# prestodb/presto

Measured on AMD Instinct MI355X. Metric: tpch_lineitem_rows_per_sec, higher is better.
Workload: dtype f64; 1 GPU; TPC-H SF100 Q1 & Q3 on 1xMI355X - one step = one Q1 pass + one Q3 pass, columns resident in HBM; query=q1+q3, rows_per_gpu=1200075804, mode=f64

## Files before the change

### include/presto_gpu.h

```cpp
#ifndef PRESTO_GPU_H
#define PRESTO_GPU_H
#include <stdint.h>

#ifdef __cplusplus
extern "C" {
#endif

#define PG_ABI_VERSION 1

typedef int32_t pg_status;
#define PG_OK 0
#define PG_ERR (-1)
const char* pg_last_error(void);

pg_status pg_device_count(int32_t* out);
pg_status pg_device_sync(void);
pg_status pg_device_malloc(int64_t bytes, void** out);
pg_status pg_device_free(void* p);
pg_status pg_memcpy_h2d(void* dst, const void* src, int64_t bytes);
pg_status pg_memcpy_d2h(void* dst, const void* src, int64_t bytes);
pg_status pg_memcpy_d2d(void* dst, const void* src, int64_t bytes);
double pg_last_hot_kernel_ms(void);
double pg_hot_max_ms(void);
void pg_hot_reset(void);
int64_t pg_q1_fast_launches(void);

typedef enum {
    PG_T_U8 = 0,
    PG_T_I32 = 1,
    PG_T_I64 = 2,
    PG_T_F64 = 3,
    PG_T_I128 = 5,
    PG_T_VARBIN = 4,
} pg_type;

typedef struct {
    int32_t tag;
    int32_t on_device;
    void* data;
    const uint8_t* null_mask;
    const int32_t* offsets;
    const int32_t* dict_ids;
    int32_t dict_n;
} pg_col;

typedef struct {
    int64_t n_rows;
    int32_t n_cols;
    pg_col cols[32];
} pg_page;


typedef enum { PG_CMP_LT = 0, PG_CMP_LE, PG_CMP_GT, PG_CMP_GE, PG_CMP_EQ,
               PG_CMP_NE,
               PG_CMP_CONTAINS, PG_CMP_PREFIX,
               PG_CMP_CONTAINS2, PG_CMP_NOT_CONTAINS2,
               PG_CMP_IS_NULL, PG_CMP_IS_NOT_NULL } pg_cmp;

typedef struct {
    int32_t col;
    int32_t op;
    int64_t ival;
    double dval;
    char sval[40];
    int32_t slen;
    int32_t rhs_col;
} pg_pred;

typedef enum {
    PG_PROJ_IDENT = 0,
    PG_PROJ_DISC_PRICE = 1,
    PG_PROJ_CHARGE = 2,
    PG_PROJ_MUL = 3,
    PG_PROJ_DIV = 4,
    PG_PROJ_KEYSHL = 5,
    PG_PROJ_SHR = 6,
    PG_PROJ_SUBDIV = 7,
    PG_PROJ_KEYSHL_DIV = 8,
} pg_proj_kind;

typedef struct {
    int32_t kind;
    int32_t a, b, c;
} pg_proj;

typedef enum {
    PG_AGG_COUNT = 0,
    PG_AGG_SUM_F64 = 1,
    PG_AGG_SUM_DEC = 2,
    PG_AGG_SUM_I64 = 3,
    PG_AGG_MIN = 4,
    PG_AGG_MAX = 5,
} pg_agg_func;

typedef struct {
    int32_t func;
    pg_proj proj;
    int32_t dec_scale;
} pg_agg;

typedef enum {
    PG_OP_FILTER_PROJECT = 1,
    PG_OP_HASH_AGG_SMALL = 2,
    PG_OP_HASH_BUILD = 3,
    PG_OP_LOOKUP_JOIN = 4,
    PG_OP_TOPN = 5,
    PG_OP_PARTITION = 6,
    PG_OP_GROUPBY_MULTI = 7,
    PG_OP_ORDER_BY = 8,
    PG_OP_WINDOW = 10,
} pg_op_kind;

#define PG_MAX_PRED 8
#define PG_MAX_AGG 8
#define PG_MAX_KEYVALS 8

typedef struct {
    int32_t n_preds;
    pg_pred preds[PG_MAX_PRED];
    int32_t n_proj;
    pg_proj proj[16];
    int64_t semijoin_table;
    int32_t semijoin_col;
    int32_t semijoin_anti;
} pg_plan_filter_project;

typedef struct {
    int32_t n_preds;
    pg_pred preds[PG_MAX_PRED];
    int32_t n_keys;
    int32_t key_col[2];
    int32_t n_vals[2];
    uint8_t key_vals[2][PG_MAX_KEYVALS];
    int32_t n_aggs;
    pg_agg aggs[PG_MAX_AGG];
    int32_t drop_unlisted_keys;
} pg_plan_hash_agg_small;

typedef struct {
    int32_t n_preds;
    pg_pred preds[PG_MAX_PRED];
    int32_t key_col;
    int64_t semijoin_table;
    int32_t semijoin_col;
    int32_t n_payload;
    int32_t payload_col[4];
    int64_t capacity_hint;
    int32_t key_set_only;
    int32_t dense_array;
    int64_t payload_lookup_table;
    int32_t payload_lookup_key_col;
    int32_t agg_table;
    int32_t pack_bits;
    int32_t fill_x10;
    int64_t bitmap_max_key;
    int32_t range_group;
    int32_t dense_payload_bias;
} pg_plan_hash_build;

#define PG_JOIN_INNER 0
#define PG_JOIN_PROBE_OUTER 4
#define PG_JOIN_LOOKUP_OUTER 5
#define PG_JOIN_FULL_OUTER 6

typedef struct {
    int64_t table;
    int32_t n_preds;
    pg_pred preds[PG_MAX_PRED];
    int32_t key_col;
    int32_t mode;
    int32_t n_emit;
    int32_t emit_probe_cols[8];
    pg_proj proj;
    int32_t dec_scale;
    int64_t table2;
    int32_t table2_key_col;
    int32_t n_group_vals;
    uint8_t group_vals[8];
// ... 110 lines not shown
```

### presto_amd/csrc/kernels.hip

```cpp
#include <hip/hip_runtime.h>
#include <stdio.h>
#include <stdlib.h>
#include <string.h>
#include <map>
#include <vector>
#include <algorithm>
#include <type_traits>
#include <stdexcept>
#include <string>

#include "../../include/presto_gpu.h"
#include "fixed128.h"
#include "sortkey.h"

static __thread char g_err[512];
extern "C" const char* pg_last_error(void) { return g_err; }
static pg_status seterr(const char* msg)
{
    snprintf(g_err, sizeof(g_err), "%s", msg);
    return PG_ERR;
}
#define CHK(x)                                                          \
    do {                                                                \
        hipError_t e_ = (x);                                            \
        if (e_ != hipSuccess) {                                         \
            snprintf(g_err, sizeof(g_err), "%s:%d %s", __FILE__,        \
                     __LINE__, hipGetErrorString(e_));                  \
            return PG_ERR;                                              \
        }                                                               \
    } while (0)
#define CHKV(x)                                                         \
    do {                                                                \
        hipError_t e_ = (x);                                            \
        if (e_ != hipSuccess) {                                         \
            snprintf(g_err, sizeof(g_err), "%s:%d %s", __FILE__,        \
                     __LINE__, hipGetErrorString(e_));                  \
            throw std::runtime_error(g_err);                            \
        }                                                               \
    } while (0)

static hipStream_t g_stream = nullptr;
static bool g_have_gpu = false;
static pg_status ensure_gpu()
{
    static int state = 0;
    if (state == 0) {
        int n = 0;
        hipError_t e = hipGetDeviceCount(&n);
        if (e != hipSuccess || n == 0) {
            state = -1;
        } else {
            if (hipStreamCreateWithFlags(&g_stream, hipStreamNonBlocking) !=
                hipSuccess)
                state = -1;
            else
                state = 1;
        }
    }
    g_have_gpu = state == 1;
    if (state != 1)
        return seterr("presto_gpu: no AMD GPU available — this library has "
                      "no CPU fallback");
    return PG_OK;
}

extern "C" pg_status pg_device_count(int32_t* out)
{
    int n = 0;
    if (hipGetDeviceCount(&n) != hipSuccess) n = 0;
    *out = n;
    return PG_OK;
}
extern "C" pg_status pg_device_sync(void)
{
    if (ensure_gpu()) return PG_ERR;
    CHK(hipDeviceSynchronize());
    return PG_OK;
}
extern "C" pg_status pg_device_malloc(int64_t bytes, void** out)
{
    if (ensure_gpu()) return PG_ERR;
    CHK(hipMalloc(out, (size_t)bytes));
    return PG_OK;
}
extern "C" pg_status pg_device_free(void* p)
{
    if (ensure_gpu()) return PG_ERR;
    CHK(hipFree(p));
    return PG_OK;
}
extern "C" pg_status pg_memcpy_h2d(void* d, const void* s, int64_t n)
{
    if (ensure_gpu()) return PG_ERR;
    CHK(hipMemcpy(d, s, (size_t)n, hipMemcpyHostToDevice));
    return PG_OK;
}
extern "C" pg_status pg_memcpy_d2h(void* d, const void* s, int64_t n)
{
    if (ensure_gpu()) return PG_ERR;
    CHK(hipMemcpy(d, s, (size_t)n, hipMemcpyDeviceToHost));
    return PG_OK;
}
extern "C" pg_status pg_memcpy_d2d(void* d, const void* s, int64_t n)
{
    if (ensure_gpu()) return PG_ERR;
    CHK(hipMemcpy(d, s, (size_t)n, hipMemcpyDeviceToDevice));
    return PG_OK;
}

static double g_last_hot_ms = 0.0;
static double g_hot_max_ms = 0.0;
static hipEvent_t g_ev0, g_ev1;
static bool g_ev_init = false;
static void hot_begin()
{
    hipError_t e;
    if (!g_ev_init) {
        e = hipEventCreate(&g_ev0);
        e = hipEventCreate(&g_ev1);
        g_ev_init = true;
    }
    e = hipEventRecord(g_ev0, g_stream);
    (void)e;
}
static void hot_end()
{
    hipError_t e;
    e = hipEventRecord(g_ev1, g_stream);
    e = hipEventSynchronize(g_ev1);
    float ms = 0;
    e = hipEventElapsedTime(&ms, g_ev0, g_ev1);
    (void)e;
    g_last_hot_ms = ms;
    if (ms > g_hot_max_ms) g_hot_max_ms = ms;
}
extern "C" double pg_last_hot_kernel_ms(void) { return g_last_hot_ms; }
extern "C" double pg_hot_max_ms(void) { return g_hot_max_ms; }
extern "C" void pg_hot_reset(void) { g_hot_max_ms = 0.0; }
static int64_t g_q1_fast_launches = 0;
extern "C" int64_t pg_q1_fast_launches(void) { return g_q1_fast_launches; }

#define WAVE 64
#define FT_NBLOCKS 4096
#define FT_NTHREADS 256
#define FT_VL ((int64_t)FT_NBLOCKS * FT_NTHREADS)
static const int64_t TBL_EMPTY = INT64_MIN;

__device__ __host__ inline uint8_t d_tbl_tag(uint64_t h)
{
    return (uint8_t)((h >> 56) | 1);
}

__device__ inline double d_load_f64(const pg_col& c, int64_t i)
{
    switch (c.tag) {
        case PG_T_F64: return ((const double*)c.data)[i];
        case PG_T_I64: return (double)((const int64_t*)c.data)[i];
        case PG_T_I32: return (double)((const int32_t*)c.data)[i];
        default: return (double)((const uint8_t*)c.data)[i];
    }
}
__device__ inline int64_t d_load_i64(const pg_col& c, int64_t i)
{
    switch (c.tag) {
        case PG_T_I64: return ((const int64_t*)c.data)[i];
        case PG_T_I32: return (int64_t)((const int32_t*)c.data)[i];
        case PG_T_U8: return (int64_t)((const uint8_t*)c.data)[i];
        default: return (int64_t)((const double*)c.data)[i];
    }
}

__device__ inline int32_t d_find(const uint8_t* d, int32_t n,
                                 const char* pat, int32_t len,
                                 int32_t from)
{
    if (len <= 0) return from <= n ? from : -1;
    const uint8_t c0 = (uint8_t)pat[0];
    const uint32_t c4 = 0x01010101u * c0;
    int32_t last = n - len;
    int32_t s = from;
    for (; s + 3 <= last; ) {
        uint32_t w;
        memcpy(&w, d + s, 4);
        uint32_t x = w ^ c4;
        uint32_t t = (x - 0x01010101u) & ~x & 0x80808080u;
        if (!t) {
            s += 4;
            continue;
        }
        for (int k = 0; k < 4; k++, s++) {
            if (((w >> (8 * k)) & 0xff) != c0) continue;
            bool e = true;
            for (int j = 1; j < len; j++)
                e = e && d[s + j] == (uint8_t)pat[j];
            if (e) return s;
        }
    }
    for (; s <= last; s++) {
        if (d[s] != c0) continue;
        bool e = true;
        for (int j = 1; j < len; j++)
            e = e && d[s + j] == (uint8_t)pat[j];
        if (e) return s;
    }
    return -1;
}

template <bool NULL_TESTS = true>
__device__ inline bool d_eval_preds(const pg_page& pg, const pg_pred* preds,
                                    int n_preds, int64_t i)
{
    for (int p = 0; p < n_preds; p++) {
        const pg_pred& pr = preds[p];
        const pg_col& c = pg.cols[pr.col];
        if constexpr (NULL_TESTS) {
            if (pr.op >= PG_CMP_IS_NULL) {
                const bool is_null = c.null_mask && c.null_mask[i];
                if (is_null != (pr.op == PG_CMP_IS_NULL)) return false;
                continue;
            }
        }
        if (c.null_mask && c.null_mask[i]) return false;
        bool ok;
        if (c.tag == PG_T_VARBIN) {
            int64_t e = c.dict_ids ? (int64_t)c.dict_ids[i] : i;
            int32_t b0 = c.offsets[e], b1 = c.offsets[e + 1];
            const uint8_t* d = (const uint8_t*)c.data + b0;
            int32_t n = b1 - b0;
            if (pr.op == PG_CMP_CONTAINS) {
                ok = d_find(d, n, pr.sval, pr.slen, 0) >= 0;
            } else if (pr.op == PG_CMP_PREFIX) {
                bool e = pr.slen <= n;
                for (int j = 0; e && j < pr.slen; j++)
                    e = d[j] == (uint8_t)pr.sval[j];
                ok = e;
            } else if (pr.op == PG_CMP_CONTAINS2 ||
                       pr.op == PG_CMP_NOT_CONTAINS2) {
                int32_t la = pr.slen, lb = (int32_t)pr.ival;
                int32_t a = d_find(d, n, pr.sval, la, 0);
                bool m = a >= 0 &&
                         d_find(d, n, pr.sval + la, lb, a + la) >= 0;
                ok = (pr.op == PG_CMP_CONTAINS2) ? m : !m;
            } else {
                bool eq = n == pr.slen;
                for (int j = 0; eq && j < pr.slen; j++)
                    eq = d[j] == (uint8_t)pr.sval[j];
                ok = pr.op == PG_CMP_EQ ? eq : !eq;
            }
        } else if (c.tag == PG_T_F64) {
            double v = ((const double*)c.data)[i];
            double x;
            if (pr.rhs_col > 0) {
                const pg_col& rc = pg.cols[pr.rhs_col - 1];
                if (rc.null_mask && rc.null_mask[i]) return false;
                x = d_load_f64(rc, i) + pr.dval;
            } else {
                x = pr.dval;
            }
            switch (pr.op) {
                case PG_CMP_LT: ok = v < x; break;
                case PG_CMP_LE: ok = v <= x; break;
                case PG_CMP_GT: ok = v > x; break;
                case PG_CMP_GE: ok = v >= x; break;
                case PG_CMP_EQ: ok = v == x; break;
                default: ok = v != x; break;
            }
        } else {
            int64_t v = d_load_i64(c, i);
            int64_t x;
            if (pr.rhs_col > 0) {
                const pg_col& rc = pg.cols[pr.rhs_col - 1];
                if (rc.null_mask && rc.null_mask[i]) return false;
                x = d_load_i64(rc, i) + pr.ival;
            } else {
                x = pr.ival;
            }
            switch (pr.op) {
                case PG_CMP_LT: ok = v < x; break;
                case PG_CMP_LE: ok = v <= x; break;
                case PG_CMP_GT: ok = v > x; break;
                case PG_CMP_GE: ok = v >= x; break;
                case PG_CMP_EQ: ok = v == x; break;
                default: ok = v != x; break;
            }
        }
        if (!ok) return false;
    }
    return true;
}

__device__ inline double d_eval_proj_f64(const pg_page& pg, const pg_proj& p,
                                         int64_t i)
{
// ... 835 lines not shown
    int64_t i = (int64_t)blockIdx.x * blockDim.x + threadIdx.x;
    int64_t stride = (int64_t)gridDim.x * blockDim.x;
    for (; i < n; i += stride) {
        int64_t key = in_keys[i];
        if (kbits) {
            if ((uint64_t)(key - 1) >= (uint64_t)bmax) {
                atomicAdd(bm_err, 1ull);
                continue;
            }
            d_kbit_set(kbits, key);
        }
        uint64_t h = pg_murmur3_finalize(pg_bigint_hash(key));
        int64_t s = (int64_t)(h & (uint64_t)mask);
        for (;;) {
            int64_t old = atomicCAS((unsigned long long*)&keys[s],
                                    (unsigned long long)TBL_EMPTY,
                                    (unsigned long long)key);
            if (old == TBL_EMPTY || old == key) {
                if (tags) tags[s] = d_tbl_tag(h);
                int32_t prev = atomicExch(&head[s], (int32_t)i);
                next[i] = prev;
                break;
            }
            s = (s + 1) & mask;
        }
    }
}

__device__ inline int64_t d_probe_next(int64_t s, int64_t lmask)
{
    return (s & ~lmask) | ((s + 1) & lmask);
}

__device__ inline int64_t d_tbl_find_tagged(const int64_t* keys,
                                            const uint8_t* tags,
                                            int64_t mask, int64_t lmask,
                                            int32_t pbits, int64_t key);

struct direct_payloads {
    void* ptr[4];
    int32_t tag[4];
    int32_t src[4];
    int32_t n;
};
__global__ __launch_bounds__(256) void k_tbl_insert_direct(
    pg_page pg, pg_plan_hash_build plan, const int64_t* set_keys,
    int64_t set_mask, const int64_t* lu_keys, const uint8_t* lu_tags,
    int64_t lu_mask, int64_t lu_lmask, const uint8_t* lu_payload,
    int64_t* keys, uint8_t* tags, direct_payloads dp, int64_t mask,
    unsigned long long* inserted, unsigned long long* overflow,
    unsigned long long* pack_err, unsigned long long* kbits, int64_t bmax,
    unsigned long long* bm_err)
{
    const int32_t pbits = plan.pack_bits;
    int64_t i = (int64_t)blockIdx.x * blockDim.x + threadIdx.x;
    int64_t stride = (int64_t)gridDim.x * blockDim.x;
    int64_t my_inserted = 0, my_overflow = 0, my_packerr = 0;
    for (; i < pg.n_rows; i += stride) {
        if (!d_eval_preds<false>(pg, plan.preds, plan.n_preds, i)) continue;
        uint8_t plv = 0;
        if (lu_payload) {
            int64_t k2 =
                d_load_i64(pg.cols[plan.payload_lookup_key_col], i);
            int64_t sl2;
            if (lu_keys) {
                sl2 = d_tbl_find_tagged(lu_keys, lu_tags, lu_mask,
                                        lu_lmask, 0, k2);
            } else {
                sl2 = (k2 >= 1 && k2 <= lu_mask) ? k2 - 1 : -1;
            }
            if (sl2 < 0) continue;
            plv = lu_payload[sl2];
        }
        if (set_keys) {
            int64_t sk = d_load_i64(pg.cols[plan.semijoin_col], i);
            bool found;
            if (set_mask < 0) {
                found = sk >= 1 && sk <= -set_mask &&
                        ((const uint8_t*)set_keys)[sk - 1];
            } else {
                found = false;
                uint64_t h = pg_murmur3_finalize(pg_bigint_hash(sk));
                int64_t s = (int64_t)(h & (uint64_t)set_mask);
                for (;;) {
                    int64_t k = set_keys[s];
                    if (k == sk) { found = true; break; }
                    if (k == TBL_EMPTY) break;
                    s = (s + 1) & set_mask;
                }
            }
            if (!found) continue;
        }
        int64_t key = d_load_i64(pg.cols[plan.key_col], i);
        int64_t word = key;
        if (pbits) {
            int64_t pay0 = lu_payload
                               ? (int64_t)plv
                               : d_load_i64(pg.cols[dp.src[0]], i);
            if (key < 0 || key >= (1ll << (63 - pbits)) || pay0 < 0 ||
                pay0 >= (1ll << pbits)) {
                my_packerr++;
                continue;
            }
            word = (key << pbits) | pay0;
        }
        if (kbits) {
            if ((uint64_t)(key - 1) >= (uint64_t)bmax) {
                atomicAdd(bm_err, 1ull);
                continue;
            }
            d_kbit_set(kbits, key);
        }
        uint64_t h = pg_murmur3_finalize(pg_bigint_hash(key));
        int64_t s = (int64_t)(h & (uint64_t)mask);
        int64_t tries = 0;
        for (;;) {
            int64_t old = atomicCAS((unsigned long long*)&keys[s],
                                    (unsigned long long)TBL_EMPTY,
                                    (unsigned long long)word);
            if (old == TBL_EMPTY || old == word) {
                if (old == TBL_EMPTY) {
                    my_inserted++;
                    if (tags) tags[s] = d_tbl_tag(h);
                }
                if (pbits) break;
                if (lu_payload && dp.n >= 1)
                    ((uint8_t*)dp.ptr[0])[s] = plv;
                for (int o = lu_payload ? 1 : 0; o < dp.n; o++) {
                    const pg_col& c = pg.cols[dp.src[o]];
                    switch (dp.tag[o]) {
                        case PG_T_U8:
                            ((uint8_t*)dp.ptr[o])[s] =
                                (uint8_t)d_load_i64(c, i);
                            break;
                        case PG_T_I32:
                            ((int32_t*)dp.ptr[o])[s] =
                                (int32_t)d_load_i64(c, i);
                            break;
                        case PG_T_I64:
                            ((int64_t*)dp.ptr[o])[s] = d_load_i64(c, i);
                            break;
                        default:
                            ((double*)dp.ptr[o])[s] = d_load_f64(c, i);
                    }
                }
                break;
            }
            if (++tries > mask) {
                my_overflow++;
                break;
            }
            s = (s + 1) & mask;
        }
    }
    my_inserted = d_bfly_i64(my_inserted);
    my_overflow = d_bfly_i64(my_overflow);
    my_packerr = d_bfly_i64(my_packerr);
    if ((threadIdx.x & 63) == 0) {
        if (my_inserted) atomicAdd(inserted, (unsigned long long)my_inserted);
        if (my_overflow) atomicAdd(overflow, (unsigned long long)my_overflow);
        if (my_packerr) atomicAdd(pack_err, (unsigned long long)my_packerr);
    }
}

#define SCAT_TILE 8192
#define SCAT_MAXP 256

struct build_row {
    int64_t key;
    int64_t pay[4];
};

__device__ inline int d_build_eval(
    const pg_page& pg, const pg_plan_hash_build& plan,
    const int64_t* set_keys, int64_t set_mask, const int64_t* lu_keys,
    const uint8_t* lu_tags, int64_t lu_mask, int64_t lu_lmask,
    const uint8_t* lu_payload, const direct_payloads& dp, int64_t i,
    bool want_pay, build_row* out)
{
    if (!d_eval_preds<false>(pg, plan.preds, plan.n_preds, i)) return 0;
    uint8_t plv = 0;
    if (lu_payload) {
        int64_t k2 = d_load_i64(pg.cols[plan.payload_lookup_key_col], i);
        int64_t sl2;
        if (lu_keys)
            sl2 = d_tbl_find_tagged(lu_keys, lu_tags, lu_mask, lu_lmask,
                                    0, k2);
        else
            sl2 = (k2 >= 1 && k2 <= lu_mask) ? k2 - 1 : -1;
        if (sl2 < 0) return 0;
        plv = lu_payload[sl2];
        out->pay[0] = (int64_t)plv;
    }
    if (set_keys) {
        int64_t sk = d_load_i64(pg.cols[plan.semijoin_col], i);
        bool found;
        if (set_mask < 0) {
            found = sk >= 1 && sk <= -set_mask &&
                    ((const uint8_t*)set_keys)[sk - 1];
        } else {
            found = false;
            uint64_t h = pg_murmur3_finalize(pg_bigint_hash(sk));
            int64_t s = (int64_t)(h & (uint64_t)set_mask);
            for (;;) {
                int64_t k = set_keys[s];
                if (k == sk) { found = true; break; }
                if (k == TBL_EMPTY) break;
                s = (s + 1) & set_mask;
            }
        }
        if (!found) return 0;
    }
    out->key = d_load_i64(pg.cols[plan.key_col], i);
    if (want_pay) {
        if (lu_payload && dp.n >= 1) out->pay[0] = (int64_t)plv;
        for (int o = lu_payload ? 1 : 0; o < dp.n; o++) {
            const pg_col& c = pg.cols[dp.src[o]];
            if (dp.tag[o] == PG_T_F64) {
                double v = d_load_f64(c, i);
                int64_t b;
                memcpy(&b, &v, 8);
                out->pay[o] = b;
            } else {
                out->pay[o] = d_load_i64(c, i);
            }
        }
    }
    return 1;
}

__global__ __launch_bounds__(256) void k_part_scatter(
    pg_page pg, pg_plan_hash_build plan, const int64_t* set_keys,
    int64_t set_mask, const int64_t* lu_keys, const uint8_t* lu_tags,
    int64_t lu_mask, int64_t lu_lmask, const uint8_t* lu_payload,
    direct_payloads dp, int64_t mask, int32_t capp_bits, int32_t P,
    int64_t* stage, unsigned long long* cursor, int64_t cap_stage_rows,
    int32_t r_words, unsigned long long* stage_ovf)
{
    __shared__ unsigned int cnt[SCAT_MAXP];
    __shared__ unsigned int c2[SCAT_MAXP];
    __shared__ unsigned long long gbase[SCAT_MAXP];
    __shared__ unsigned int rowp[SCAT_TILE];
    const int64_t n = pg.n_rows;
    for (int64_t t0 = (int64_t)blockIdx.x * SCAT_TILE; t0 < n;
         t0 += (int64_t)gridDim.x * SCAT_TILE) {
        const int64_t t1 = t0 + SCAT_TILE < n ? t0 + SCAT_TILE : n;
        for (int p = threadIdx.x; p < P; p += 256) {
            cnt[p] = 0;
            c2[p] = 0;
        }
        __syncthreads();
        for (int64_t i = t0 + threadIdx.x; i < t1; i += 256) {
            build_row r;
            r.pay[0] = 0;
            unsigned int tagw = 0;
            if (d_build_eval(pg, plan, set_keys, set_mask, lu_keys,
                             lu_tags, lu_mask, lu_lmask, lu_payload, dp,
                             i, false, &r)) {
                uint64_t h = pg_murmur3_finalize(pg_bigint_hash(r.key));
                int p = (int)((h & (uint64_t)mask) >> capp_bits);
                atomicAdd(&cnt[p], 1u);
                tagw = (unsigned int)(p + 1) |
                       ((unsigned int)(uint8_t)r.pay[0] << 16);
            }
            rowp[i - t0] = tagw;
        }
        __syncthreads();
        for (int p = threadIdx.x; p < P; p += 256) {
            if (cnt[p]) {
                unsigned long long b =
                    atomicAdd(&cursor[p], (unsigned long long)cnt[p]);
                gbase[p] = b;
                if (b + cnt[p] > (unsigned long long)cap_stage_rows)
                    atomicAdd(stage_ovf, 1ull);
            }
        }
        __syncthreads();
        for (int64_t i = t0 + threadIdx.x; i < t1; i += 256) {
            unsigned int tagw = rowp[i - t0];
            if (!tagw) continue;
            int p = (int)(tagw & 0xffffu) - 1;
            unsigned long long row = gbase[p] + atomicAdd(&c2[p], 1u);
            if (row >= (unsigned long long)cap_stage_rows) continue;
            int64_t* rec = stage +
                ((int64_t)p * cap_stage_rows + (int64_t)row) * r_words;
            rec[0] = d_load_i64(pg.cols[plan.key_col], i);
            const bool lu = lu_payload != nullptr;
            if (lu && dp.n >= 1) rec[1] = (int64_t)(tagw >> 16);
            for (int o = lu ? 1 : 0; o < dp.n; o++) {
                const pg_col& c = pg.cols[dp.src[o]];
                if (dp.tag[o] == PG_T_F64) {
                    double v = d_load_f64(c, i);
                    int64_t b;
                    memcpy(&b, &v, 8);
                    rec[1 + o] = b;
                } else {
                    rec[1 + o] = d_load_i64(c, i);
                }
            }
        }
        __syncthreads();
    }
}

__device__ inline void d_grid_barrier(unsigned long long* bar,
                                      unsigned long long target)
// ... 2758 lines not shown
            case 4 * 16 + 4: launch2<4, 4>(sp.pg); break;
            case 4 * 16 + 6: launch2<4, 6>(sp.pg); break;
            case 4 * 16 + 8: launch2<4, 8>(sp.pg); break;
            case 7 * 16 + 2: launch2<7, 2>(sp.pg); break;
            case 7 * 16 + 4: launch2<7, 4>(sp.pg); break;
            case 7 * 16 + 6: launch2<7, 6>(sp.pg); break;
            case 7 * 16 + 8: launch2<7, 8>(sp.pg); break;
            case 9 * 16 + 2: launch2<9, 2>(sp.pg); break;
            case 9 * 16 + 4: launch2<9, 4>(sp.pg); break;
            case 9 * 16 + 6: launch2<9, 6>(sp.pg); break;
            default: launch2<9, 8>(sp.pg); break;
        }
        hot_end();
        if (!sp.bufs.empty()) CHKV(hipStreamSynchronize(g_stream));
    }
    void finish() override
    {
        int nm = na * maxg;
        DevBuf out_f, out_hi, out_lo;
        out_f.alloc(nm * 8);
        out_hi.alloc(nm * 8);
        out_lo.alloc(nm * 8);
        if (dec)
            hipLaunchKernelGGL(k_agg_small_finish<true>, dim3(nm),
                               dim3(WAVE), 0, g_stream, nullptr,
                               (int64_t*)partials.p, nm, nullptr,
                               (int64_t*)out_hi.p, (uint64_t*)out_lo.p,
                               funcs());
        else
            hipLaunchKernelGGL(k_agg_small_finish<false>, dim3(nm),
                               dim3(WAVE), 0, g_stream,
                               (double*)partials.p, nullptr, nm,
                               (double*)out_f.p, nullptr, nullptr,
                               funcs());
        std::vector<double> hf(nm);
        std::vector<int64_t> hhi(nm);
        std::vector<uint64_t> hlo(nm);
        unsigned long long hbad[2] = {0, 0};
        CHKV(hipMemcpyAsync(hf.data(), out_f.p, nm * 8, hipMemcpyDeviceToHost,
                            g_stream));
        CHKV(hipMemcpyAsync(hhi.data(), out_hi.p, nm * 8,
                            hipMemcpyDeviceToHost, g_stream));
        CHKV(hipMemcpyAsync(hlo.data(), out_lo.p, nm * 8,
                            hipMemcpyDeviceToHost, g_stream));
        CHKV(hipMemcpyAsync(hbad, bad_ptr(), 16, hipMemcpyDeviceToHost,
                            g_stream));
        CHKV(hipStreamSynchronize(g_stream));
        if (hbad[0])
            throw std::runtime_error(
                "group key value outside plan enumeration");
        if (hbad[1])
            throw std::runtime_error(
                "bigint/decimal SUM overflow (Math.addExact semantics, "
                "LongSumAggregation.java:33-37)");
        for (int a = 0; a < user_aggs; a++)
            if (dec && plan.aggs[a].func == PG_AGG_SUM_I64)
                for (int g = 0; g < n_groups; g++) {
                    int64_t hi = hhi[a * maxg + g];
                    int64_t lo = (int64_t)hlo[a * maxg + g];
                    if (hi != (lo < 0 ? -1 : 0))
                        throw std::runtime_error(
                            "BIGINT sum overflow (Math.addExact semantics, "
                            "LongSumAggregation.java:33-37)");
                }
        int ic = user_aggs;
        auto cnt_of = [&](int g) -> int64_t {
            return dec ? (int64_t)hlo[ic * maxg + g]
                       : (int64_t)hf[ic * maxg + g];
        };
        int n_out = 0;
        for (int g = 0; g < n_groups; g++)
            if (cnt_of(g) > 0) n_out++;
        OutPage op;
        op.pg.n_rows = n_out;
        int nc = 0;
        auto add_host_col = [&](int tag) {
            op.host.emplace_back((size_t)n_out * type_size(tag));
            op.pg.cols[nc].tag = tag;
            op.pg.cols[nc].on_device = 0;
            op.pg.cols[nc].data = op.host.back().data();
            op.pg.cols[nc].null_mask = nullptr;
            return nc++;
        };
        int c_k0 = plan.n_keys >= 1 ? add_host_col(PG_T_U8) : -1;
        int c_k1 = plan.n_keys == 2 ? add_host_col(PG_T_U8) : -1;
        std::vector<int> agg_col(user_aggs);
        std::vector<int> agg_col2(user_aggs, -1);
        for (int a = 0; a < user_aggs; a++) {
            if (dec && plan.aggs[a].func != PG_AGG_COUNT) {
                agg_col[a] = add_host_col(PG_T_I64);
                agg_col2[a] = add_host_col(PG_T_I64);
            } else if (plan.aggs[a].func == PG_AGG_COUNT) {
                agg_col[a] = add_host_col(PG_T_I64);
            } else {
                agg_col[a] = add_host_col(PG_T_F64);
            }
        }
        op.pg.n_cols = nc;
        int row = 0;
        for (int g = 0; g < n_groups; g++) {
            if (cnt_of(g) <= 0) continue;
            int i0 = plan.n_keys == 2 ? g / plan.n_vals[1] : g;
            int i1 = plan.n_keys == 2 ? g % plan.n_vals[1] : 0;
            if (c_k0 >= 0)
                ((uint8_t*)op.pg.cols[c_k0].data)[row] = plan.key_vals[0][i0];
            if (c_k1 >= 0)
                ((uint8_t*)op.pg.cols[c_k1].data)[row] =
                    plan.key_vals[1][i1];
            for (int a = 0; a < user_aggs; a++) {
                if (plan.aggs[a].func == PG_AGG_COUNT) {
                    ((int64_t*)op.pg.cols[agg_col[a]].data)[row] = cnt_of(g);
                } else if (dec) {
                    ((int64_t*)op.pg.cols[agg_col[a]].data)[row] =
                        hhi[a * maxg + g];
                    ((int64_t*)op.pg.cols[agg_col2[a]].data)[row] =
                        (int64_t)hlo[a * maxg + g];
                } else {
                    ((double*)op.pg.cols[agg_col[a]].data)[row] =
                        hf[a * maxg + g];
                }
            }
            row++;
        }
        outq.push_back(std::move(op));
    }
};

static int persistent_grid()
{
    static int nb = 0;
    if (!nb) {
        hipDeviceProp_t p{};
        int cus = 0;
        if (hipGetDeviceProperties(&p, 0) == hipSuccess)
            cus = p.multiProcessorCount;
        if (cus <= 0) cus = 64;
        if (cus > 256) cus = 256;
        nb = cus * 4;
        const char* e = getenv("PG_PART_NB");
        if (e && atoi(e) > 0) nb = atoi(e);
    }
    return nb;
}

struct BuildOp : Op {
    pg_plan_hash_build plan;
    int64_t tbl = -1;
    std::unique_ptr<Table> t;
    int64_t cap_rows = 0;
    DevBuf counters;
    bool part = false;
    int32_t P = 1, Kact = 1, capp_bits = 0;
    DevBuf stage, cursorb, barb;
    void init()
    {
        t.reset(new Table());
        t->key_set_only = plan.key_set_only != 0;
        if (plan.dense_array || plan.agg_table)
            for (int p = 0; p < plan.n_preds && p < PG_MAX_PRED; p++)
                if (plan.preds[p].op >= PG_CMP_IS_NULL)
                    throw std::runtime_error(
                        "IS NULL / IS NOT NULL predicates are not "
                        "supported on dense_array and agg_table builds "
                        "(filter ahead of the build, or use a chained "
                        "build)");
        if (plan.range_group) {
            if (plan.capacity_hint <= 0)
                throw std::runtime_error(
                    "range_group needs capacity_hint = max key");
            t->range_group = true;
            t->slot_payloads = true;
            t->cap = plan.capacity_hint;
            t->mask = t->cap - 1;
            t->local_mask = t->mask;
            return;
        }
        if (plan.dense_array) {
            if (plan.n_payload != 1 && !plan.key_set_only)
                throw std::runtime_error(
                    "dense_array needs one u8 payload (or key_set_only)");
            t->dense = true;
            t->cap = plan.capacity_hint;
            t->payload.emplace_back();
            t->ptag.push_back(PG_T_U8);
            t->dense_alloc_pending = true;
            if (plan.key_set_only) {
                t->payload.back().alloc((size_t)t->cap);
                t->payload.back().zero();
                t->dense_alloc_pending = false;
            }
            return;
        }
        if (plan.agg_table) {
            t->slot_payloads = true;
            if (plan.pack_bits) {
                if (plan.n_payload != 1 || plan.pack_bits < 1 ||
                    plan.pack_bits > 32)
                    throw std::runtime_error(
                        "pack_bits needs exactly one payload and "
                        "1..32 bits");
                t->pack_bits = plan.pack_bits;
            }
            int64_t mult10 = plan.fill_x10 >= 11 ? plan.fill_x10 : 20;
            if (const char* em = getenv("PG_CAP_X10"))
                if (atoi(em) >= 11) mult10 = atoi(em);
            int64_t cap = next_pow2(plan.capacity_hint * mult10 / 10 + 16);
            t->cap = cap;
            t->mask = cap - 1;
            t->local_mask = cap - 1;
            t->keys.alloc((size_t)cap * 8);
            int64_t part_min = 512ll << 20;
            if (const char* ep = getenv("PG_PART_MIN_SLOTS"))
                if (atoll(ep) > 0) part_min = atoll(ep);
            part = cap >= part_min;
            bool always_hit = plan.fill_x10 >= 11 && plan.fill_x10 < 20;
            if (!always_hit && (part || cap >= (64ll << 20))) {
                t->tags.alloc((size_t)cap);
                if (!part) t->tags.zero();
            }
            counters.alloc(40);
            counters.zero();
            if (plan.bitmap_max_key > 0) {
                t->bmax = plan.bitmap_max_key;
                t->kbits.alloc((size_t)((t->bmax >> 6) + 1) * 8);
                t->kbits.zero();
            }
            if (part) {
                P = 256;
                while (cap / P < (64ll << 10)) P >>= 1;
                int64_t slot_bytes = 8 + (t->tags.p ? 1 : 0) +
                                     8ll * plan.n_payload;
                int64_t region_bytes = cap / P * slot_bytes;
                Kact = (int32_t)((128ll << 20) / region_bytes);
                if (Kact < 1) Kact = 1;
                if (Kact > P) Kact = P;
                const char* ek = getenv("PG_PART_K");
                if (ek && atoi(ek) > 0) {
                    Kact = atoi(ek);
                    if (Kact > P) Kact = P;
                }
                int64_t cap_p = cap / P;
                capp_bits = 0;
                while ((1ll << capp_bits) < cap_p) capp_bits++;
                t->local_mask = cap_p - 1;
                int32_t r_words = 1 + plan.n_payload;
                stage.alloc((size_t)cap * r_words * 8);
                cursorb.alloc((size_t)P * 8);
                cursorb.zero();
                barb.alloc(8);
                barb.zero();
            } else {
                hipLaunchKernelGGL(k_tbl_init, dim3(1024), dim3(256), 0,
                                   g_stream, (int64_t*)t->keys.p, nullptr,
                                   cap);
            }
            for (int i = 0; i < plan.n_payload; i++) {
                t->payload.emplace_back();
                t->ptag.push_back(-1);
                t->payload.back().alloc(
                    plan.pack_bits ? 1 : (size_t)cap * 8);
            }
            return;
        }
        cap_rows = plan.capacity_hint > 16 ? plan.capacity_hint : 16;
        t->key_rows.alloc((size_t)cap_rows * 8);
        for (int i = 0; i < plan.n_payload; i++) {
            t->payload.emplace_back();
            t->ptag.push_back(-1);
            t->payload.back().alloc((size_t)cap_rows * 8);
        }
    }
    void grow(int64_t need)
    {
        if (need <= cap_rows) return;
        int64_t nc = cap_rows;
        while (nc < need) nc *= 2;
        DevBuf nk;
        nk.alloc((size_t)nc * 8);
        CHKV(hipMemcpyAsync(nk.p, t->key_rows.p, (size_t)t->n_rows * 8,
                            hipMemcpyDeviceToDevice, g_stream));
        t->key_rows = std::move(nk);
        for (size_t i = 0; i < t->payload.size(); i++) {
            DevBuf np;
            np.alloc((size_t)nc * 8);
            CHKV(hipMemcpyAsync(np.p, t->payload[i].p,
                                (size_t)t->n_rows *
                                    (t->ptag[i] >= 0
                                         ? type_size(t->ptag[i])
                                         : 8),
                                hipMemcpyDeviceToDevice, g_stream));
            t->payload[i] = std::move(np);
        }
        cap_rows = nc;
    }
    const Table* semi_table()
    {
        if (plan.semijoin_table < 0) return nullptr;
        std::lock_guard<std::mutex> lk(g_mu);
        auto it = g_tables.find(plan.semijoin_table);
        if (it == g_tables.end())
            throw std::runtime_error("semijoin table not found");
        return it->second.get();
    }
    void add_input(const pg_page* in) override
    {
        if (plan.range_group)
            throw std::runtime_error(
                "range_group tables take no build input (the domain is "
                "the key range itself)");
        StagedPage sp;
        sp.stage(in);
        for (int i = 0; i < plan.n_payload; i++)
            if (t->ptag[i] < 0)
                t->ptag[i] = (plan.agg_table &&
                              plan.payload_lookup_table > 0 && i == 0)
                                 ? PG_T_U8
                                 : sp.pg.cols[plan.payload_col[i]].tag;
        if (plan.dense_array) {
            if (plan.semijoin_table > 0)
                throw std::runtime_error(
                    "dense_array builds do not evaluate semijoins — "
                    "pre-filter with a FILTER_PROJECT semijoin instead");
            if (sp.pg.cols[plan.key_col].tag != PG_T_I64 ||
                (!plan.key_set_only && !plan.payload_lookup_table &&
                 sp.pg.cols[plan.payload_col[0]].tag != PG_T_U8 &&
                 sp.pg.cols[plan.payload_col[0]].tag != PG_T_I32))
                throw std::runtime_error(
                    "dense_array expects I64 keys and a U8/I32 payload");
            int32_t ptag =
                plan.key_set_only || plan.payload_lookup_table
                    ? PG_T_U8
                    : sp.pg.cols[plan.payload_col[0]].tag;
            if (t->dense_alloc_pending) {
                t->ptag[0] = ptag;
                t->payload[0].alloc((size_t)t->cap *
                                    (ptag == PG_T_I32 ? 4 : 1));
                t->payload[0].zero();
                t->dense_alloc_pending = false;
            } else if (t->ptag[0] != ptag) {
                throw std::runtime_error(
                    "dense_array payload tag changed across pages");
            }
            if (plan.payload_lookup_table > 0) {
                const Table* lu;
                {
                    std::lock_guard<std::mutex> lk(g_mu);
                    auto it = g_tables.find(plan.payload_lookup_table);
                    if (it == g_tables.end() || !it->second->dense ||
                        it->second->ptag[0] != PG_T_U8)
                        throw std::runtime_error(
                            "dense fill lookup needs a dense u8 table");
                    lu = it->second.get();
                }
                hipLaunchKernelGGL(
                    k_dense_fill_lu, dim3(2048), dim3(256), 0, g_stream,
                    sp.pg, plan, (const uint8_t*)lu->payload[0].p,
                    lu->cap, (uint8_t*)t->payload[0].p, t->cap);
            } else if (ptag == PG_T_I32)
                hipLaunchKernelGGL(
                    k_dense_fill32, dim3(2048), dim3(256), 0, g_stream,
                    sp.pg, plan,
                    (const int32_t*)sp.pg.cols[plan.payload_col[0]].data,
                    (int32_t*)t->payload[0].p, t->cap);
            else
                hipLaunchKernelGGL(
                    k_dense_fill, dim3(2048), dim3(256), 0, g_stream,
                    sp.pg, plan,
                    plan.key_set_only
                        ? nullptr
                        : (const uint8_t*)
                              sp.pg.cols[plan.payload_col[0]].data,
                    (uint8_t*)t->payload[0].p, t->cap);
            CHKV(hipStreamSynchronize(g_stream));
            return;
        }
        if (plan.agg_table) {
            const Table* semi = semi_table();
            const Table* lu = nullptr;
            if (plan.payload_lookup_table > 0) {
                std::lock_guard<std::mutex> lk(g_mu);
                auto it = g_tables.find(plan.payload_lookup_table);
                if (it == g_tables.end() ||
                    !(it->second->slot_payloads || it->second->dense) ||
                    it->second->ptag.empty() ||
                    it->second->ptag[0] != PG_T_U8)
                    throw std::runtime_error(
                        "payload_lookup_table must be an agg_table or "
                        "dense_array with a u8 payload");
                lu = it->second.get();
            }
            direct_payloads dp{};
            dp.n = plan.n_payload;
            for (int o = 0; o < dp.n; o++) {
                dp.ptr[o] = t->payload[o].p;
                dp.tag[o] = lu && o == 0 ? PG_T_U8 : t->ptag[o];
                dp.src[o] = plan.payload_col[o];
            }
            if (part) {
                hot_begin();
                hipLaunchKernelGGL(
                    k_part_scatter, dim3(2048), dim3(256), 0, g_stream,
                    sp.pg, plan, set_ptr(semi), set_mask_of(semi),
                    lu && !lu->dense ? (const int64_t*)lu->keys.p
                                     : nullptr,
                    lu && !lu->dense ? (const uint8_t*)lu->tags.p
                                     : nullptr,
                    lu ? (lu->dense ? lu->cap : lu->mask) : 0,
                    lu ? (lu->dense ? lu->cap : lu->local_mask) : 0,
                    lu ? (const uint8_t*)lu->payload[0].p : nullptr, dp,
                    t->mask, capp_bits, P, (int64_t*)stage.p,
                    (unsigned long long*)cursorb.p, t->cap / P,
                    1 + plan.n_payload,
                    (unsigned long long*)counters.p + 2);
                hot_end();
                CHKV(hipStreamSynchronize(g_stream));
                return;
            }
            hot_begin();
            hipLaunchKernelGGL(k_tbl_insert_direct, dim3(4096), dim3(256),
                               0, g_stream, sp.pg, plan, set_ptr(semi),
                               set_mask_of(semi),
                               lu && !lu->dense
                                   ? (const int64_t*)lu->keys.p
                                   : nullptr,
                               lu && !lu->dense
                                   ? (const uint8_t*)lu->tags.p
                                   : nullptr,
                               lu ? (lu->dense ? lu->cap : lu->mask) : 0,
                               lu ? (lu->dense ? lu->cap : lu->local_mask)
                                  : 0,
                               lu ? (const uint8_t*)lu->payload[0].p
                                  : nullptr,
                               (int64_t*)t->keys.p,
                               (uint8_t*)t->tags.p, dp, t->mask,
                               (unsigned long long*)counters.p,
                               (unsigned long long*)counters.p + 1,
                               (unsigned long long*)counters.p + 3,
                               (unsigned long long*)t->kbits.p, t->bmax,
                               (unsigned long long*)counters.p + 4);
            hot_end();
            CHKV(hipStreamSynchronize(g_stream));
            return;
        }
        pg_plan_filter_project fp{};
        fp.n_preds = plan.n_preds;
        memcpy(fp.preds, plan.preds, sizeof(fp.preds));
        fp.n_proj = 1 + plan.n_payload;
        fp.proj[0].kind = PG_PROJ_IDENT;
        fp.proj[0].a = plan.key_col;
        for (int i = 0; i < plan.n_payload; i++) {
            fp.proj[1 + i].kind = PG_PROJ_IDENT;
            fp.proj[1 + i].a = plan.payload_col[i];
        }
        const Table* semi = nullptr;
        if (plan.semijoin_table >= 0) {
            std::lock_guard<std::mutex> lk(g_mu);
            auto it = g_tables.find(plan.semijoin_table);
            if (it == g_tables.end())
                throw std::runtime_error("semijoin table not found");
            semi = it->second.get();
        }
        int64_t chunk = sel_chunk(sp.pg.n_rows);
        SelResult r =
            sel_count(sp.pg, fp, semi, plan.semijoin_col, chunk);
        grow(t->n_rows + r.n);
        emit_outs outs{};
        outs.n = fp.n_proj;
        outs.ptr[0] = (int8_t*)t->key_rows.p + t->n_rows * 8;
        outs.tag[0] = PG_T_I64;
        for (int i = 0; i < plan.n_payload; i++) {
            outs.ptr[1 + i] = (int8_t*)t->payload[i].p +
                              t->n_rows * type_size(t->ptag[i]);
            outs.tag[1 + i] = t->ptag[i];
        }
        if (sp.pg.cols[plan.key_col].tag != PG_T_I64)
            throw std::runtime_error("build key must be an I64 column");
        sel_emit(sp.pg, fp, semi, plan.semijoin_col, chunk, r, outs);
        t->n_rows += r.n;
    }
    void finish() override
    {
        if (plan.dense_array || plan.range_group) {
            std::lock_guard<std::mutex> lk(g_mu);
            tbl = g_next_table++;
            g_tables[tbl] = std::move(t);
            return;
        }
        if (plan.agg_table) {
            if (part) {
                direct_payloads dp{};
                dp.n = plan.n_payload;
                for (int o = 0; o < dp.n; o++) {
                    dp.ptr[o] = t->payload[o].p;
                    dp.tag[o] = (plan.payload_lookup_table > 0 && o == 0)
                                    ? PG_T_U8
                                    : t->ptag[o];
                }
                static int use_bar = -1;
                if (use_bar < 0) {
                    const char* eb = getenv("PG_PART_BARRIER");
                    use_bar = eb ? atoi(eb) : 0;
                }
                hot_begin();
                if (!use_bar) {
                    hipLaunchKernelGGL(k_tbl_init, dim3(1024), dim3(256),
                                       0, g_stream, (int64_t*)t->keys.p,
                                       nullptr, t->cap);
                    if (t->tags.p)
                        CHKV(hipMemsetAsync(t->tags.p, 0, t->tags.sz,
                                            g_stream));
                }
                hipLaunchKernelGGL(k_part_insert,
                                   dim3(use_bar ? persistent_grid()
                                                : 4096), dim3(256), 0,
                                   g_stream, (const int64_t*)stage.p,
                                   (const unsigned long long*)cursorb.p,
                                   t->cap / P, 1 + plan.n_payload,
                                   (int64_t*)t->keys.p,
                                   (uint8_t*)t->tags.p, dp, t->cap / P, P,
                                   Kact, use_bar, plan.pack_bits,
                                   (unsigned long long*)barb.p,
                                   (unsigned long long*)counters.p,
                                   (unsigned long long*)counters.p + 1,
                                   (unsigned long long*)counters.p + 3,
                                   (unsigned long long*)t->kbits.p,
                                   t->bmax,
                                   (unsigned long long*)counters.p + 4);
                hot_end();
                CHKV(hipStreamSynchronize(g_stream));
                stage.free();
                cursorb.free();
                barb.free();
            }
            unsigned long long c[5];
            CHKV(hipMemcpy(c, counters.p, 40, hipMemcpyDeviceToHost));
            if (c[4])
                throw std::runtime_error(
                    "bitmap_max_key violated: build key outside "
                    "[1, bitmap_max_key]");
            if (c[3])
                throw std::runtime_error(
                    "pack_bits violated: key or payload outside the "
                    "declared bit ranges");
            if (c[2])
                throw std::runtime_error(
                    "partition staging overflow (unexpected hash skew): "
                    "raise capacity_hint");
            if (c[1])
                throw std::runtime_error(
                    "agg table overflow: capacity_hint too small");
            if ((int64_t)c[0] * 100 > t->cap * 85)
                throw std::runtime_error(
                    "agg table fill exceeded 0.85: raise capacity_hint");
            t->n_rows = (int64_t)c[0];
            std::lock_guard<std::mutex> lk(g_mu);
            tbl = g_next_table++;
            g_tables[tbl] = std::move(t);
            return;
        }
        int64_t cap = next_pow2(t->n_rows * 2 + 16);
        t->cap = cap;
        t->mask = cap - 1;
        t->local_mask = cap - 1;
        t->keys.alloc((size_t)cap * 8);
        if (!t->key_set_only) {
            t->head.alloc((size_t)cap * 4);
            t->next.alloc((size_t)(t->n_rows ? t->n_rows : 1) * 4);
// ... 2441 lines not shown
```

Measured before the change: 112.5 billion rows/s.

## Add staged vectorized hash-build insert kernel for packed single-payload builds

Adds a specialized hash-table insert kernel for builds with packed keys and one payload. Each thread handles four consecutive rows using vector nontemporal loads, and all four CAS operations are issued before any collision chains are walked, so the atomics overlap. It is used by default (can be disabled with an environment variable) when predicates are simple int32 compares and the columns are aligned and non-null. The aim is to speed up the Q3 hash build's memory access, at the cost of a second code path whose checks and counters must match the general insert kernel.

```diff
diff --git a/include/presto_gpu.h b/include/presto_gpu.h
--- a/include/presto_gpu.h
+++ b/include/presto_gpu.h
@@ -24,6 +24,7 @@
 double pg_hot_max_ms(void);
 void pg_hot_reset(void);
 int64_t pg_q1_fast_launches(void);
+int64_t pg_build_staged_launches(void);
 
 typedef enum {
     PG_T_U8 = 0,
diff --git a/presto_amd/csrc/kernels.hip b/presto_amd/csrc/kernels.hip
--- a/presto_amd/csrc/kernels.hip
+++ b/presto_amd/csrc/kernels.hip
@@ -139,6 +139,11 @@
 extern "C" void pg_hot_reset(void) { g_hot_max_ms = 0.0; }
 static int64_t g_q1_fast_launches = 0;
 extern "C" int64_t pg_q1_fast_launches(void) { return g_q1_fast_launches; }
+static int64_t g_build_staged_launches = 0;
+extern "C" int64_t pg_build_staged_launches(void)
+{
+    return g_build_staged_launches;
+}
 
 #define WAVE 64
 #define FT_NBLOCKS 4096
@@ -1280,6 +1285,197 @@
             }
             s = (s + 1) & mask;
         }
+    }
+    my_inserted = d_bfly_i64(my_inserted);
+    my_overflow = d_bfly_i64(my_overflow);
+    my_packerr = d_bfly_i64(my_packerr);
+    if ((threadIdx.x & 63) == 0) {
+        if (my_inserted) atomicAdd(inserted, (unsigned long long)my_inserted);
+        if (my_overflow) atomicAdd(overflow, (unsigned long long)my_overflow);
+        if (my_packerr) atomicAdd(pack_err, (unsigned long long)my_packerr);
+    }
+}
+
+#define BS_R 4
+#define BS_TILE (256 * BS_R)
+struct staged_args {
+    const int32_t* pc[2];
+    int64_t pval[2];
+    int32_t pop[2];
+    int32_t n_preds;
+    const int64_t* sk;
+    const uint8_t* flags;
+    int64_t nflags;
+    const int64_t* lk;
+    const uint8_t* lu;
+    int64_t lucap;
+    const int64_t* key;
+    const void* pay;
+    int32_t pay_tag;
+    int32_t pay_pred;
+    int64_t n;
+};
+__device__ inline bool d_cmp_i64(int32_t op, int64_t v, int64_t x)
+{
+    switch (op) {
+        case PG_CMP_LT: return v < x;
+        case PG_CMP_LE: return v <= x;
+        case PG_CMP_GT: return v > x;
+        case PG_CMP_GE: return v >= x;
+        case PG_CMP_EQ: return v == x;
+        default: return v != x;
+    }
+}
+__device__ inline void d_bs_load_i32(const int32_t* p, int64_t base,
+                                     int64_t n, bool full, int64_t* out)
+{
+    typedef int vi4 __attribute__((ext_vector_type(4)));
+    if (full) {
+        vi4 v = __builtin_nontemporal_load((const vi4*)(p + base));
+#pragma unroll
+        for (int j = 0; j < BS_R; j++) out[j] = v[j];
+    } else {
+#pragma unroll
+        for (int j = 0; j < BS_R; j++)
+            out[j] = base + j < n ? p[base + j] : 0;
+    }
+}
+__device__ inline void d_bs_load_i64(const int64_t* p, int64_t base,
+                                     int64_t n, bool full, int64_t* out)
+{
+    typedef long vl2 __attribute__((ext_vector_type(2)));
+    if (full) {
+#pragma unroll
+        for (int j = 0; j < BS_R; j += 2) {
+            vl2 v = __builtin_nontemporal_load((const vl2*)(p + base + j));
+            out[j] = v[0];
+            out[j + 1] = v[1];
+        }
+    } else {
+#pragma unroll
+        for (int j = 0; j < BS_R; j++)
+            out[j] = base + j < n ? p[base + j] : 0;
+    }
+}
+__device__ inline void d_bs_probe(int64_t* keys, uint8_t* tags,
+                                  int64_t mask, uint64_t h, int64_t s,
+                                  int64_t word, int64_t old,
+                                  int64_t& my_inserted, int64_t& my_overflow)
+{
+    int64_t tries = 0;
+    for (;;) {
+        if (old == TBL_EMPTY || old == word) {
+            if (old == TBL_EMPTY) {
+                my_inserted++;
+                if (tags) tags[s] = d_tbl_tag(h);
+            }
+            return;
+        }
+        if (++tries > mask) {
+            my_overflow++;
+            return;
+        }
+        s = (s + 1) & mask;
+        old = atomicCAS((unsigned long long*)&keys[s],
+                        (unsigned long long)TBL_EMPTY,
+                        (unsigned long long)word);
+    }
+}
+__global__ __launch_bounds__(256) void k_tbl_insert_staged(
+    staged_args a, int32_t pbits, int64_t* keys, uint8_t* tags,
+    int64_t mask, unsigned long long* inserted,
+    unsigned long long* overflow, unsigned long long* pack_err,
+    unsigned long long* kbits, int64_t bmax, unsigned long long* bm_err)
+{
+    const int64_t n = a.n;
+    const int64_t n_tiles = (n + BS_TILE - 1) / BS_TILE;
+    int64_t my_inserted = 0, my_overflow = 0, my_packerr = 0;
+    for (int64_t tile = blockIdx.x; tile < n_tiles; tile += gridDim.x) {
+        const int64_t base = tile * BS_TILE + (int64_t)threadIdx.x * BS_R;
+        const bool full = base + BS_R <= n;
+        int64_t pv[2][BS_R] = {}, skv[BS_R] = {}, lkv[BS_R] = {}, kv[BS_R];
+        if (a.n_preds > 0) d_bs_load_i32(a.pc[0], base, n, full, pv[0]);
+        if (a.n_preds > 1) d_bs_load_i32(a.pc[1], base, n, full, pv[1]);
+        if (a.sk) d_bs_load_i64(a.sk, base, n, full, skv);
+        if (a.lk) d_bs_load_i64(a.lk, base, n, full, lkv);
+        d_bs_load_i64(a.key, base, n, full, kv);
+        bool ok[BS_R];
+#pragma unroll
+        for (int j = 0; j < BS_R; j++) {
+            ok[j] = base + j < n;
+            if (a.n_preds > 0)
+                ok[j] = ok[j] && d_cmp_i64(a.pop[0], pv[0][j], a.pval[0]);
+            if (a.n_preds > 1)
+                ok[j] = ok[j] && d_cmp_i64(a.pop[1], pv[1][j], a.pval[1]);
+            if (a.lk) ok[j] = ok[j] && lkv[j] >= 1 && lkv[j] <= a.lucap;
+            if (a.sk) ok[j] = ok[j] && skv[j] >= 1 && skv[j] <= a.nflags;
+        }
+        uint8_t fl[BS_R], plv[BS_R];
+        int64_t pay[BS_R];
+#pragma unroll
+        for (int j = 0; j < BS_R; j++) {
+            fl[j] = 1;
+            plv[j] = 0;
+            pay[j] = 0;
+            if (!ok[j]) continue;
+            if (a.sk) fl[j] = a.flags[skv[j] - 1];
+            if (a.lk) plv[j] = a.lu[lkv[j] - 1];
+            else if (a.pay_pred < 0) {
+                if (a.pay_tag == PG_T_I32)
+                    pay[j] = ((const int32_t*)a.pay)[base + j];
+                else if (a.pay_tag == PG_T_U8)
+                    pay[j] = ((const uint8_t*)a.pay)[base + j];
+                else
+                    pay[j] = ((const int64_t*)a.pay)[base + j];
+            }
+        }
+#pragma unroll
+        for (int j = 0; j < BS_R; j++) {
+            ok[j] = ok[j] && fl[j] != 0;
+            if (a.lk) pay[j] = plv[j];
+            else if (a.pay_pred >= 0)
+                pay[j] = a.pay_pred ? pv[1][j] : pv[0][j];
+        }
+        int64_t word[BS_R];
+#pragma unroll
+        for (int j = 0; j < BS_R; j++) {
+            word[j] = 0;
+            if (!ok[j]) continue;
+            const int64_t key = kv[j];
+            if (key < 0 || key >= (1ll << (63 - pbits)) || pay[j] < 0 ||
+                pay[j] >= (1ll << pbits)) {
+                my_packerr++;
+                ok[j] = false;
+                continue;
+            }
+            if (kbits) {
+                if ((uint64_t)(key - 1) >= (uint64_t)bmax) {
+                    atomicAdd(bm_err, 1ull);
+                    ok[j] = false;
+                    continue;
+                }
+                d_kbit_set(kbits, key);
+            }
+            word[j] = (key << pbits) | pay[j];
+        }
+        uint64_t h[BS_R];
+        int64_t old[BS_R];
+#pragma unroll
+        for (int j = 0; j < BS_R; j++) {
+            h[j] = pg_murmur3_finalize(pg_bigint_hash(kv[j]));
+            old[j] = 0;
+            if (ok[j])
+                old[j] = atomicCAS(
+                    (unsigned long long*)&keys[h[j] & (uint64_t)mask],
+                    (unsigned long long)TBL_EMPTY,
+                    (unsigned long long)word[j]);
+        }
+#pragma unroll
+        for (int j = 0; j < BS_R; j++)
+            if (ok[j])
+                d_bs_probe(keys, tags, mask, h[j],
+                           (int64_t)(h[j] & (uint64_t)mask), word[j], old[j],
+                           my_inserted, my_overflow);
     }
     my_inserted = d_bfly_i64(my_inserted);
     my_overflow = d_bfly_i64(my_overflow);
@@ -4344,6 +4540,63 @@
     bool part = false;
     int32_t P = 1, Kact = 1, capp_bits = 0;
     DevBuf stage, cursorb, barb;
+    bool staged = true;
+    bool staged_fit(const pg_page& pg, const Table* semi, const Table* lu,
+                    staged_args* sa) const
+    {
+        auto vec_i64 = [](const pg_col& c) {
+            return c.tag == PG_T_I64 && !c.null_mask &&
+                   ((uintptr_t)c.data & 15) == 0;
+        };
+        if (!staged || plan.pack_bits <= 0 || plan.n_payload != 1)
+            return false;
+        if (plan.n_preds < 0 || plan.n_preds > 2) return false;
+        staged_args a{};
+        a.n = pg.n_rows;
+        a.n_preds = plan.n_preds;
+        for (int p = 0; p < plan.n_preds; p++) {
+            const pg_pred& pr = plan.preds[p];
+            const pg_col& c = pg.cols[pr.col];
+            if (pr.rhs_col != 0 || pr.op < PG_CMP_LT || pr.op > PG_CMP_NE ||
+                c.tag != PG_T_I32 || c.null_mask ||
+                ((uintptr_t)c.data & 15) != 0)
+                return false;
+            a.pc[p] = (const int32_t*)c.data;
+            a.pval[p] = pr.ival;
+            a.pop[p] = pr.op;
+        }
+        const pg_col& kc = pg.cols[plan.key_col];
+        if (!vec_i64(kc)) return false;
+        a.key = (const int64_t*)kc.data;
+        if (semi) {
+            const pg_col& sc = pg.cols[plan.semijoin_col];
+            if (!semi->dense || semi->ptag.empty() ||
+                semi->ptag[0] != PG_T_U8 || !vec_i64(sc))
+                return false;
+            a.sk = (const int64_t*)sc.data;
+            a.flags = (const uint8_t*)semi->payload[0].p;
+            a.nflags = semi->cap;
+        }
+        a.pay_pred = -1;
+        if (lu) {
+            const pg_col& lc = pg.cols[plan.payload_lookup_key_col];
+            if (!lu->dense || !vec_i64(lc)) return false;
+            a.lk = (const int64_t*)lc.data;
+            a.lu = (const uint8_t*)lu->payload[0].p;
+            a.lucap = lu->cap;
+        } else {
+            const pg_col& pc = pg.cols[plan.payload_col[0]];
+            if (pc.tag != PG_T_I32 && pc.tag != PG_T_U8 &&
+                pc.tag != PG_T_I64)
+                return false;
+            a.pay = pc.data;
+            a.pay_tag = pc.tag;
+            for (int p = 0; p < plan.n_preds; p++)
+                if (plan.preds[p].col == plan.payload_col[0]) a.pay_pred = p;
+        }
+        *sa = a;
+        return true;
+    }
     void init()
     {
         t.reset(new Table());
@@ -4405,6 +4658,9 @@
             if (const char* ep = getenv("PG_PART_MIN_SLOTS"))
                 if (atoll(ep) > 0) part_min = atoll(ep);
             part = cap >= part_min;
+            staged = true;
+            if (const char* es = getenv("PG_BUILD_STAGED"))
+                staged = atoi(es) != 0;
             bool always_hit = plan.fill_x10 >= 11 && plan.fill_x10 < 20;
             if (!always_hit && (part || cap >= (64ll << 20))) {
                 t->tags.alloc((size_t)cap);
@@ -4605,6 +4861,26 @@
                     1 + plan.n_payload,
                     (unsigned long long*)counters.p + 2);
                 hot_end();
+                CHKV(hipStreamSynchronize(g_stream));
+                return;
+            }
+            staged_args sa;
+            if (staged_fit(sp.pg, semi, lu, &sa)) {
+                int64_t tiles = (sa.n + BS_TILE - 1) / BS_TILE;
+                int grid = (int)(tiles < 4096 ? (tiles > 0 ? tiles : 1)
+                                              : 4096);
+                hot_begin();
+                hipLaunchKernelGGL(
+                    k_tbl_insert_staged, dim3(grid), dim3(256), 0, g_stream,
+                    sa, plan.pack_bits, (int64_t*)t->keys.p,
+                    (uint8_t*)t->tags.p, t->mask,
+                    (unsigned long long*)counters.p,
+                    (unsigned long long*)counters.p + 1,
+                    (unsigned long long*)counters.p + 3,
+                    (unsigned long long*)t->kbits.p, t->bmax,
+                    (unsigned long long*)counters.p + 4);
+                hot_end();
+                g_build_staged_launches++;
                 CHKV(hipStreamSynchronize(g_stream));
                 return;
             }
```

Result: faster. 120.5 billion rows/s (median of 6 runs) (+7.1%).
